# irmen/synthesizer

Measured on AMD Instinct MI355X. Metric: Msamples/sec mixed to stereo bus, 1024-voice additive @48kHz, higher is better.
Workload: dtype f64

## Files before the change

### synthesizer_amd/csrc/common.hpp

```cpp
#pragma once
#include <hip/hip_runtime.h>
#include <stdint.h>
#include <stddef.h>
#include <mutex>
#include <string>
#include "../../include/synthhip.h"

struct sh_buf {
    void*  ptr;
    size_t bytes;
    bool   owner;
    size_t cap = 0;
};

namespace sh {

struct PendingCombine {
    const void* parts = nullptr;
    uint32_t groups = 0, nframes = 0;
    void*    o32 = nullptr;
    void*    o64 = nullptr;
    void*    o16 = nullptr;
    double   scale = 0.0;
    const void* gen_valid = nullptr;
};

struct State {
    bool        initialized = false;
    int         device = -1;
    hipStream_t stream = nullptr;
    hipStream_t comm_stream = nullptr;
    hipEvent_t  ev_start = nullptr, ev_stop = nullptr;
    void*       scratch = nullptr;
    size_t      scratch_bytes = 0;
    int         last_mixdown_fused = 0;
    int         quantise_round = 0;
    int*        flag = nullptr;
    int*        flag_host = nullptr;
    void*       trig = nullptr;
    int         pending_total = 0;
    int         open_runs = 0;
    hipStream_t stream2 = nullptr;
    hipEvent_t  ev_join = nullptr;
    hipEvent_t  ev_aux = nullptr;
    hipEvent_t  ev_prep = nullptr;
    hipEvent_t  ev_sync = nullptr;
    bool        aux_busy = false;
};

State& state();

struct Knobs {
    bool no_speculation = false;
    bool no_overlap = false;
    bool no_split = false;
    bool no_seg = false;
    bool no_tiles = false;
    int  self = 0;
    bool no_ladder = false;
    bool no_period = false;
    int  period_chunks = 0;
    int  rt_cus = 0;
    int  seq_align = 0;
    bool no_small_pipeline = false;
    int  variant = 0;
    int  groups = 0;
    int  pool_fill = -1;
};
const Knobs& knobs();
void load_knobs();

struct Counters {
    uint64_t device_allocs = 0;
    uint64_t device_frees = 0;
    uint64_t stream_syncs = 0;
    uint64_t pool_hits = 0;
    uint64_t segmented_launches = 0, tiled_launches = 0, tiled_predicted = 0;
};
Counters& counters();
std::recursive_mutex& api_mutex();
#define SH_API_LOCK() std::lock_guard<std::recursive_mutex> sh_api_lock__(sh::api_mutex())
int  set_error(int code, const char* fmt, ...);
int  hip_error(hipError_t e, const char* what);
int  ensure_scratch(size_t bytes);
int  pool_alloc(size_t bytes, void** ptr, size_t* cap);
void pool_free(void* ptr, size_t cap);
void pool_trim();
struct Pooled {
    void*  ptr = nullptr;
    size_t cap = 0;
};
int  join_streams();
int  grow_pooled(Pooled& p, size_t bytes);
void release_pooled(Pooled& p);
int  flush_pending();
void free_render_buffers();
bool fold_owed_into(const void* p, size_t bytes);
inline bool has_pending() { return state().pending_total != 0 || state().aux_busy || state().open_runs != 0; }
int  bus_finalize_on(hipStream_t st, const double* in, size_t nvalues, float* out);

int bind_thread_to_device();
#define SH_REQUIRE_INIT_KEEP_PENDING()                                                 \
    SH_API_LOCK();                                                                     \
    do {                                                                               \
        if (!sh::state().initialized)                                                  \
            return sh::set_error(SH_ERR_NOTINIT, "sh_init() has not been called");     \
        { int rc_bind__ = sh::bind_thread_to_device(); if (rc_bind__) return rc_bind__; } \
    } while (0)

#define SH_REQUIRE_INIT()                                                              \
    SH_API_LOCK();                                                                     \
// ... 55 lines not shown
```

### synthesizer_amd/csrc/devmath.hpp

```cpp
#pragma once
#include <stdint.h>
#include <math.h>

#if defined(__HIPCC__)
#define SH_HD __host__ __device__ __forceinline__
#else
#define SH_HD static inline
#endif

namespace shm {

constexpr double PI_1 = 0x1.921fb54442d18p+1;
constexpr double PI_2 = 0x1.1a62633145c07p-53;
constexpr double PI_3 = -0x1.f1976b7ed8fbcp-109;
constexpr double INV_PI = 0.3183098861837907;
constexpr double PIO2_1 = 0x1.921fb54442d18p+0;
constexpr double PIO2_2 = 0x1.1a62633145c07p-54;
constexpr double PIO2_3 = -0x1.f1976b7ed8fbcp-110;
constexpr double TWO_OVER_PI = 0.6366197723675814;

SH_HD double flip_sign(double x, int odd) {
    union { double d; uint64_t u; } v;
    v.d = x;
    v.u ^= ((uint64_t)(odd & 1)) << 63;
// ... 56 lines not shown
    double fn = rint(t * TWO_OVER_PI);
    double r = fma(-fn, PIO2_1, t);
    r = fma(-fn, PIO2_2, r);
    r = fma(-fn, PIO2_3, r);
    int q = (int)fn;
    double z = r * r;
    double ps = -7.647163731819816e-13;
    ps = fma(ps, z, 1.6059043836821613e-10);
    ps = fma(ps, z, -2.505210838544172e-08);
    ps = fma(ps, z, 2.7557319223985893e-06);
    ps = fma(ps, z, -0.0001984126984126984);
    ps = fma(ps, z, 0.008333333333333333);
    ps = fma(ps, z, -0.16666666666666666);
    double sr = fma(r * z, ps, r);
    double pc = 4.779477332387385e-14;
    pc = fma(pc, z, -1.1470745597729725e-11);
    pc = fma(pc, z, 2.08767569878681e-09);
    pc = fma(pc, z, -2.755731922398589e-07);
    pc = fma(pc, z, 2.48015873015873e-05);
    pc = fma(pc, z, -0.001388888888888889);
    pc = fma(pc, z, 0.041666666666666664);
    pc = fma(pc, z, -0.5);
    double cr = fma(z, pc, 1.0);
    double s0 = (q & 1) ? cr : sr;
    double c0 = (q & 1) ? sr : cr;
    s = flip_sign(s0, (q >> 1) & 1);
    c = flip_sign(c0, ((q + 1) >> 1) & 1);
}

constexpr int    TRIG_N = 512;
constexpr double TRIG_STEP_1 = PI_1 / 256.0;
constexpr double TRIG_STEP_2 = PI_2 / 256.0;
constexpr double TRIG_STEP_3 = PI_3 / 256.0;
constexpr double TRIG_INV_STEP = 81.48733086305042;

struct sc_pair { double s, c; };

template <typename TablePtr>
SH_HD void sincos_tab(double t, TablePtr tab, double& s, double& c) {
    union { double d; uint64_t u; } m;
    m.d = fma(t, TRIG_INV_STEP, 6755399441055744.0);
    const double fk = m.d - 6755399441055744.0;
    double r = fma(-fk, TRIG_STEP_1, t);
    r = fma(-fk, TRIG_STEP_2, r);
    const uint32_t k = (uint32_t)m.u & (uint32_t)(TRIG_N - 1);
    const double S = tab[k].s, C = tab[k].c;
    const double z = r * r;
    const double sr = fma(r * z, fma(z, 0.008333333333333333, -0.16666666666666666), r);
    const double cr = fma(z, fma(z, 0.041666666666666664, -0.5), 1.0);
    s = fma(S, cr, C * sr);
    c = fma(C, cr, -(S * sr));
}

template <int N, typename TablePtr>
SH_HD void sincos_tab_n(const double (&t)[N], TablePtr tab, double (&s)[N], double (&c)[N]) {
    double r[N], S[N], C[N];
    for (int j = 0; j < N; ++j) {
        union { double d; uint64_t u; } m;
        m.d = fma(t[j], TRIG_INV_STEP, 6755399441055744.0);
        const double fk = m.d - 6755399441055744.0;
        const uint32_t k = (uint32_t)m.u & (uint32_t)(TRIG_N - 1);
        S[j] = tab[k].s;
        C[j] = tab[k].c;
        r[j] = fma(-fk, TRIG_STEP_2, fma(-fk, TRIG_STEP_1, t[j]));
    }
    double z[N], sr[N], cr[N];
    for (int j = 0; j < N; ++j) z[j] = r[j] * r[j];
    for (int j = 0; j < N; ++j) sr[j] = fma(z[j], 0.008333333333333333, -0.16666666666666666);
    for (int j = 0; j < N; ++j) cr[j] = fma(z[j], 0.041666666666666664, -0.5);
    for (int j = 0; j < N; ++j) sr[j] = fma(r[j] * z[j], sr[j], r[j]);
    for (int j = 0; j < N; ++j) cr[j] = fma(z[j], cr[j], 1.0);
    for (int j = 0; j < N; ++j) s[j] = fma(S[j], cr[j], C[j] * sr[j]);
    for (int j = 0; j < N; ++j) c[j] = fma(C[j], cr[j], -(S[j] * sr[j]));
}


SH_HD double saw_value(double t, double amp2, double bias) {
    double fl = floor(0.5 + t);
    return bias + amp2 * (t - fl);
}

SH_HD double square_value(double t, double amp, double bias) {
    double tr = trunc(t * 2.0);
    double h = tr * 0.5;
    bool odd = (h != rint(h)) && (fabs(tr) < 9007199254740992.0);
    return (odd ? -amp : amp) + bias;
}

SH_HD double pulse_value(double t, double pw, double amp, double bias) {
    double m = t - trunc(t);
    if (m < 0.0) m = m + 1.0;
    return ((m < pw) ? amp : -amp) + bias;
}

SH_HD double triangle_value(double t, double amp4, double bias) {
    double u = t + 0.75;
    double m = u - trunc(u);
    if (m < 0.0) m = m + 1.0;
    return amp4 * (fabs(m - 0.5) - 0.25) + bias;
}

}
```

### synthesizer_amd/csrc/osc_device.hpp

```cpp
#pragma once
#include "common.hpp"
#include "devmath.hpp"
#include "renderplan.hpp"
#include <type_traits>

namespace shosc {


constexpr uint32_t TILE_MAX_PIECES = 3;
struct alignas(64) TileRec {
    double t0, dt;
    double rc, rs;
    double ea0, ea1, eb0, eb1;
    double GL, GR;
    double tb[2], db[2];
    uint16_t split[2];
    uint16_t npieces;
    uint16_t corner;
    double pad_;
};
constexpr uint32_t TILE_WALK_PIECES = 16;
static_assert(sizeof(TileRec) == TILE_REC_BYTES && sizeof(TileRec) == 128 && offsetof(TileRec, GL) == 64 && offsetof(TileRec, tb) == 80 && offsetof(TileRec, split) == 112, "TileRec layout");
__device__ __forceinline__ double readlane_f64(double v, uint32_t src) {
    union { double d; int u[2]; } a, b;
// ... 988 lines not shown
                    if (SLOPED) {
                        const double ij = dl + (double)(f * 64);
                        accl[f] = fma(fma(ij, gls, gl), x, accl[f]);
                        accr[f] = fma(fma(ij, grs, gr), x, accr[f]);
                    } else {
                        accl[f] = fma(gl, x, accl[f]);
                        accr[f] = fma(gr, x, accr[f]);
                    }
                }
            }
        }
        return;
    }
#pragma unroll
    for (int h = 0; h < FPL; h += 2) {
        const bool two = h + 1 < FPL;
        double p0 = fma(poly[0], c0, poly[1]), p1 = fma(poly[0], c1, poly[1]);
#pragma unroll
        for (int u = 2; u < 16; ++u) {
            p0 = fma(p0, c0, poly[u]);
            if (two) p1 = fma(p1, c1, poly[u]);
        }
        const double x0 = p0 * s0;
        if (SLOPED) {
            const double i0 = dl + (double)(h * 64);
            accl[h] = fma(fma(i0, gls, gl), x0, accl[h]);
            accr[h] = fma(fma(i0, grs, gr), x0, accr[h]);
        } else {
            accl[h] = fma(gl, x0, accl[h]);
            accr[h] = fma(gr, x0, accr[h]);
        }
        if (two) {
            const double x1 = p1 * s1;
            if (SLOPED) {
                const double i1 = dl + (double)((h + 1) * 64);
                accl[h + 1 < FPL ? h + 1 : h] = fma(fma(i1, gls, gl), x1, accl[h + 1 < FPL ? h + 1 : h]);
                accr[h + 1 < FPL ? h + 1 : h] = fma(fma(i1, grs, gr), x1, accr[h + 1 < FPL ? h + 1 : h]);
            } else {
                accl[h + 1 < FPL ? h + 1 : h] = fma(gl, x1, accl[h + 1 < FPL ? h + 1 : h]);
                accr[h + 1 < FPL ? h + 1 : h] = fma(gr, x1, accr[h + 1 < FPL ? h + 1 : h]);
            }
        }
        if (h + 2 < FPL) {
            if (straddle) {
                shm::sincos_tab(theta(h + 2), trig, s0, c0);
                if (h + 3 < FPL) shm::sincos_tab(theta(h + 3), trig, s1, c1);
            } else {
                const double s2 = fma(k2, s1, -s0), c2 = fma(k2, c1, -c0);
                const double s3 = fma(k2, s2, -s1), c3 = fma(k2, c2, -c1);
                s0 = s2; c0 = c2; s1 = s3; c1 = c3;
            }
        }
    }
}

constexpr int TILE_WIN = 6;
template <typename V>
__device__ __forceinline__ V win_pick(const V (&a)[TILE_WIN], uint32_t r, V beyond) {
    V x = beyond;
#pragma unroll
    for (int k = 0; k < TILE_WIN; ++k) x = r == (uint32_t)k ? a[k] : x;
    return x;
}
__device__ __forceinline__ void prepare_tiles_wave(const BankPtrs& B, const TileSet& T, uint32_t nvoices, uint64_t start, uint32_t nframes,
                                                   uint32_t ntiles, uint32_t c, uint32_t run, const LaunchSet* recs = nullptr) {
    const uint32_t lane = threadIdx.x & 63, vi = c * 64 + lane;
    const size_t slots = (size_t)T.rec_chunks * 64;
    const uint32_t t_begin = run * TILES_PER_WAVE;
    if (t_begin >= ntiles) return;
    uint32_t t_end = t_begin + TILES_PER_WAVE;
    if (t_end > ntiles) t_end = ntiles;
    const bool valid = vi < nvoices;
    const uint64_t launch_end = start + (uint64_t)nframes;
    {
        const uint64_t span_lo = as_const(B.chunk_span)[2 * c], span_hi = as_const(B.chunk_span)[2 * c + 1];
        if (launch_end <= span_lo || start >= span_hi) {
            if (lane == 0)
                for (uint32_t t = t_begin; t < t_end; ++t) {
                    const size_t at = ((size_t)t * T.groups + c % T.groups) * T.mask_k + c / T.groups;
                    T.lean[at] = 0;
                    T.gen[at] = 0;
                }
            return;
        }
    }
    const sh_voice& v = B.voices[valid ? vi : 0];
    const int32_t v_kind = v.kind, v_dense = v.harm_dense, v_fm = v.fm_mode, v_flip = v.flip;
    const double v_bias = v.bias, amp = v.amplitude;
    const uint32_t off_c = v.seg_offset, cnt_c = v.seg_count, off_t = v.time_seg_offset, cnt_t = v.time_seg_count;
    const uint64_t onset = v.start_frame;
    const uint64_t e_na = v.env.n_attack_end, e_nd = v.env.n_decay_end, e_ns = v.env.n_sustain_end, e_nr = v.env.n_release_end;
    const double e_as = v.env.attack_slope, e_ds = v.env.decay_slope, e_sl = v.env.sustain_level, e_rs = v.env.release_slope;
    const int32_t e_on = v.env.enabled, e_tail = v.env.has_tail;
    const double bgl = (double)v.gain_l, bgr = (double)v.gain_r;
    const uint32_t hint = B.hint[valid ? vi : 0];
    asm volatile("" :: "v"(v_kind), "v"(v_dense), "v"(v_fm), "v"(v_flip), "v"(v_bias), "v"(amp), "v"(off_c), "v"(cnt_c), "v"(off_t), "v"(cnt_t),
                 "v"(onset), "v"(e_na), "v"(e_nd), "v"(e_ns), "v"(e_nr), "v"(e_as), "v"(e_ds), "v"(e_sl), "v"(e_rs), "v"(e_on), "v"(e_tail),
                 "v"(bgl), "v"(bgr), "v"(hint));
    const bool v_wave = v_kind == SH_SAWTOOTH || v_kind == SH_SQUARE || v_kind == SH_TRIANGLE || v_kind == SH_PULSE;
    const bool v_fm_sine = v_kind == SH_SINE && v_fm == SH_FM_SINE;
    const bool lean_capable = valid && v_bias == 0.0 && !v_flip &&
                              (v_fm_sine || (v_fm == SH_FM_NONE && ((v_kind == SH_HARMONICS && v_dense == 2) || v_kind == SH_SINE || v_wave)));
    const uint32_t rec_kind = v_fm_sine ? LEAN_FM : v_kind == SH_SAWTOOTH ? LEAN_SAW : v_kind == SH_SQUARE ? LEAN_SQUARE : v_kind == SH_TRIANGLE ? LEAN_TRIANGLE : v_kind == SH_PULSE ? LEAN_PULSE : LEAN_HARM;
    const bool fm = v_fm != SH_FM_NONE;
    const uint32_t off = fm ? off_t : off_c;
    const uint32_t cnt = fm ? cnt_t : cnt_c;
// ... 206 lines not shown
```

### synthesizer_amd/csrc/osc_render.hip

```cpp
#include "osc_host.hpp"
#include "osc_render_kernels.hpp"
#include "renderplan.hpp"
#include <stdlib.h>


namespace {

struct WriteRec { const char* lo; const char* hi; const sh_bank* owner; uint8_t streams; };
std::vector<WriteRec>& bank_writes() {
    static std::vector<WriteRec> v;
    return v;
}
bool overlaps_writes(const sh_bank* b, bool own, uint8_t streams, const void* p, size_t bytes) {
    if (!p) return false;
    const char* lo = (const char*)p;
    for (const WriteRec& r : bank_writes())
        if ((r.owner == b) == own && (!own || (r.streams & streams)) && lo < r.hi && r.lo < lo + bytes) return true;
    return false;
}
void note_write(const sh_bank* b, const void* p, size_t bytes, uint8_t stream_bit) {
    if (!p) return;
    const char* lo = (const char*)p;
    for (WriteRec& r : bank_writes())
        if (r.owner == b && r.lo == lo) { if (lo + bytes > r.hi) r.hi = lo + bytes; r.streams |= stream_bit; return; }
// ... 55 lines not shown
            const PendingCombine& pc = b->pending[k];
            const struct { const void* q; size_t n; } outs[3] = {{pc.o32, (size_t)pc.nframes * 8}, {pc.o64, (size_t)pc.nframes * 16}, {pc.o16, (size_t)pc.nframes * 4}};
            for (const auto& o : outs)
                if (o.q && lo < (const char*)o.q + o.n && (const char*)o.q < lo + bytes) return true;
        }
    return false;
}

int join_streams() {
    State& S = state();
    int rc = join_aux();
    if (rc) return rc;
    SH_HIP(hipEventRecord(S.ev_sync, S.stream));
    SH_HIP(hipStreamWaitEvent(S.stream2, S.ev_sync, 0));
    return SH_OK;
}

void free_render_buffers() {
    for (sh_bank* b : live_banks()) {
        for (int k = 0; k < 4; ++k) release_pooled(b->parts[k]);
        for (int k = 0; k < 2; ++k) {
            release_pooled(b->seg_block[k]);
            release_pooled(b->seg_scratch[k]);
            b->seg_cap[k] = 0;
        }
        release_pooled(b->gen_block);
        b->gen_segs = 0;
        for (int k = 0; k < sh_bank::NTILESETS; ++k) {
            release_pooled(b->tile_block[k]);
            b->tile_carved[k] = 0;
            b->tile_spec[k].valid = false;
        }
    }
}
}

struct RenderLaunch {
    sh_bank* b;
    hipStream_t st;
    shr::Call call;
    const shr::Shape& S;
    uint64_t next_start;
    uint32_t prep_wgs;
    bool use_aux;
    bool records_deferred;
    bool self_prepare;
    bool alone;
    LaunchSet cur, next;
    BusOut out;
    double2* parts;
    FoldIn fold;
    uint32_t* gen_valid;
    LaunchArgs args(const BankPtrs& P, const LaunchSet& set) const {
        return LaunchArgs{P, trig_table(), b->nvoices, S.vpg, set, call.start, call.nframes, self_prepare ? 1u : 0u, alone ? 1u : 0u};
    }
    NextArgs next_args(const LaunchSet& nx, uint32_t wgs) const { return NextArgs{nx, next_start, wgs}; }
};
static dim3 dim(shr::Grid g) { return dim3(g.x, g.y); }

static int launch_tiled(const RenderLaunch& L) {
    sh_bank* b = L.b;
    hipStream_t st = L.st;
    const shr::Shape& S = L.S;
    const shr::TiledGrids G = shr::tiled_grids(*b, S, L.call, L.next.launch != nullptr);
    int rc = SH_OK;
    const int ks = (int)(b->tile_count % sh_bank::NTILESETS);
    TileSet& T = b->tile_set[ks];
    sh_bank::TileSpec& sp = b->tile_spec[ks];
    BankPtrs P = ptrs(b);
    sh::counters().tiled_launches += 1;
    const bool predicted = shr::holds(sp, L.call, S.groups);
    if (predicted) sh::counters().tiled_predicted += 1;
    if (!predicted) {
        rc = grow_tile_set(b->tile_block[ks], T, b->tile_carved[ks], G.ntiles, b->nvoices, S.groups, (G.k1 - G.k0) * S.groups, st);
        if (rc) return rc;
        T.k0 = G.k0; T.k1 = G.k1;
        P.tiles = T;
        const LaunchSet own = launch_set(b, b->cur);
        rc = launch_prepare_tiles(st, P, T, b->nvoices, L.call.start, L.call.nframes, L.records_deferred ? &own : nullptr);
        if (rc) return rc;
    } else if (L.records_deferred) {
        rc = prepare_chunks_now(b, L.call.start, L.call.nframes, st);
        if (rc) return rc;
    }
    sp.valid = false;
    if (L.next.launch) {
        const int k2 = (int)((b->tile_count + 2) % sh_bank::NTILESETS);
        TileSet& T2 = b->tile_set[k2];
        rc = grow_tile_set(b->tile_block[k2], T2, b->tile_carved[k2], G.ntiles, b->nvoices, S.groups, (G.nk1 - G.nk0) * S.groups, st);
        if (rc) return rc;
        T2.k0 = G.nk0; T2.k1 = G.nk1;
        P.next_tiles = T2;
        P.next_ntiles = G.ntiles;
        P.next_tile_wgs = G.next_tile_wgs;
        b->tile_spec[k2] = sh_bank::TileSpec{true, L.next_start, L.call.nframes, S.groups};
    }
    P.tiles = T;
    const LaunchArgs A = L.args(P, L.cur);
    LaunchSet nx = L.next;
    if (!G.next_in_kernel) nx.launch = nullptr;
    const NextArgs N = L.next_args(nx, G.behind);
    if (G.merged) {
        if (b->tile_waveforms) hipLaunchKernelGGL((k_render_tiles<4, 8, 3, true, true>), dim(G.tiles), dim3(256), 0, st, A, N, L.fold, L.parts, L.gen_valid);
        else hipLaunchKernelGGL((k_render_tiles<4, 8, 3, false, true>), dim(G.tiles), dim3(256), 0, st, A, N, L.fold, L.parts, L.gen_valid);
    } else {
        if (b->tile_waveforms) hipLaunchKernelGGL((k_render_tiles<4, 8, 3, true, false>), dim(G.tiles), dim3(256), 0, st, A, N, L.fold, L.parts, L.gen_valid);
        else hipLaunchKernelGGL((k_render_tiles<4, 8, 4, false, false>), dim(G.tiles), dim3(256), 0, st, A, N, L.fold, L.parts, L.gen_valid);
// ... 305 lines not shown
```

### synthesizer_amd/csrc/osc_render_kernels.hpp

```cpp
#pragma once
#include "osc_device.hpp"
#include <type_traits>

namespace shosc {
struct BusOut {
    float2*   bus32;
    double2*  bus64;
    uint32_t* pcm16;
    double    pcm_scale;
};
struct FoldIn {
    const double2*  parts;
    const uint32_t* gen_valid;
    BusOut          out;
    uint32_t*       self;
};
struct LaunchArgs {
    BankPtrs              B;
    const shm::sc_pair*   trig_g;
    uint32_t              nvoices, voices_per_group;
    LaunchSet             cur;
    uint64_t              start;
    uint32_t              nframes;
    uint32_t              self_prepare;
    uint32_t              alone;
};
struct NextArgs {
    LaunchSet next;
    uint64_t  next_start;
    uint32_t  prep_wgs;
};
int launch_render_lean(int var, int kinds, bool seg, dim3 grid, hipStream_t st, const LaunchArgs& A, const NextArgs& N, const FoldIn& F, double2* parts);
int launch_render_combined(int var, int mode, dim3 grid, hipStream_t st, const LaunchArgs& A, const NextArgs& N, const FoldIn& F, double2* parts, const BusOut& out);
}

namespace {


#ifdef SH_DIAG
constexpr uint32_t DIAG_WAVES = 4096, DIAG_SLOTS = 10;
__device__ uint64_t g_diag[4 * DIAG_WAVES * DIAG_SLOTS];
__device__ __forceinline__ void diag_stamp(uint64_t start_, uint32_t nframes_, uint32_t slot) {
    const uint32_t w = (blockIdx.y * gridDim.x + blockIdx.x) * (blockDim.x >> 6) + (threadIdx.x >> 6);
    if ((threadIdx.x & 63) == 0 && w < DIAG_WAVES) {
        const uint32_t bank = (uint32_t)((double)start_ * __builtin_amdgcn_rcp((double)nframes_) + 0.5);
        uint64_t* d = g_diag + ((size_t)(bank & 3) * DIAG_WAVES + w) * DIAG_SLOTS;
        d[slot] = __builtin_amdgcn_s_memrealtime();
        if (slot == 0) {
            uint32_t hw, xcc;
            asm volatile("s_getreg_b32 %0, hwreg(HW_REG_HW_ID)" : "=s"(hw));
            asm volatile("s_getreg_b32 %0, hwreg(HW_REG_XCC_ID)" : "=s"(xcc));
            d[6] = (uint64_t)hw | ((uint64_t)xcc << 32);
            d[7] = __builtin_amdgcn_s_memtime();
            d[9] = ((uint64_t)gridDim.x << 32) | gridDim.y;
        }
        if (slot == 5) d[8] = __builtin_amdgcn_s_memtime();
    }
}
__device__ uint64_t g_diag2[64 * 8];
#define SH_STAMP(A_, slot) diag_stamp((A_).start, (A_).nframes, slot)
#else
#define SH_STAMP(A_, slot) ((void)0)
#endif

struct TileCtx {
    uint32_t lane, wave;
    uint32_t grp, ngroups;
    uint32_t tile_index, tile0, tile_last, nfr;
    uint32_t seg_off;
    uint64_t st0;
    uint32_t c0, c1;
    LaunchSet set;
    uint32_t alone;
};

template <int FPL>
__device__ __forceinline__ void tile_bounds(TileCtx& T) {
    T.tile0 = T.tile_index * (64 * FPL);
    T.tile_last = T.tile0 + 64 * FPL - 1;
    if (T.tile_last > T.nfr - 1) T.tile_last = T.nfr - 1;
}

__device__ __forceinline__ void group_chunks(TileCtx& T, const LaunchArgs& A) {
    T.c0 = (T.grp * A.voices_per_group) / 64;
    T.c1 = ((T.grp + 1) * A.voices_per_group + 63) / 64;
    const uint32_t nchunks = (A.nvoices + 63) / 64;
    if (T.c1 > nchunks) T.c1 = nchunks;
}

template <int FPL>
__device__ __forceinline__ TileCtx plain_tile(const LaunchArgs& A, uint32_t bx, uint32_t grp, uint32_t ngroups) {
    TileCtx T;
    T.lane = threadIdx.x & 63;
    T.wave = __builtin_amdgcn_readfirstlane(threadIdx.x >> 6);
    T.grp = grp;
    T.ngroups = ngroups;
    T.tile_index = bx;
    T.nfr = A.nframes;
    T.seg_off = 0;
    T.st0 = A.start;
    T.set = A.cur;
    T.alone = A.alone;
    tile_bounds<FPL>(T);
    group_chunks(T, A);
    return T;
}

template <int FPL>
__device__ __forceinline__ void enter_segment(TileCtx& T, const LaunchArgs& A) {
    uint32_t sidx = 0;
    for (;;) {
        const uint32_t n_s = A.B.seg_first[sidx + 1] - A.B.seg_first[sidx];
        const uint32_t tiles_s = (n_s + 64 * FPL - 1) / (64 * FPL);
        if (T.tile_index < tiles_s || sidx + 1 >= A.B.nseg) break;
        T.tile_index -= tiles_s;
        ++sidx;
    }
    T.seg_off = A.B.seg_first[sidx];
    T.nfr = A.B.seg_first[sidx + 1] - T.seg_off;
    T.st0 = A.start + T.seg_off;
    T.set = segment_set(A.cur, sidx, A.nvoices);
    tile_bounds<FPL>(T);
}

template <int FPL>
__device__ __forceinline__ void build_frames(const TileCtx& T, uint32_t lane_, uint32_t (&i)[FPL], double (&di)[FPL]) {
#pragma unroll
    for (int j = 0; j < FPL; ++j) {
        const uint32_t raw = T.tile0 + j * 64 + lane_;
        i[j] = raw < T.nfr ? raw : T.nfr - 1;
        di[j] = (double)i[j];
    }
}

__device__ __forceinline__ void load_trig(shm::sc_pair* trig, const shm::sc_pair* __restrict__ trig_g, uint32_t nthreads) {
    for (uint32_t k = threadIdx.x; k < shm::TRIG_N; k += nthreads) trig[k] = trig_g[k];
    __syncthreads();
}

__device__ __forceinline__ uint32_t groups_of_grid(uint32_t prep_wgs) {
    return gridDim.y - (prep_wgs ? (prep_wgs + gridDim.x - 1) / gridDim.x : 0u);
}
__device__ __forceinline__ bool prep_rows_lists(const LaunchArgs& A, const NextArgs& N, uint32_t ngroups) {
    if (!N.prep_wgs || blockIdx.y < ngroups) return false;
    const uint32_t unit = (blockIdx.y - ngroups) * gridDim.x + blockIdx.x;
    if (N.next.launch && unit < N.prep_wgs && threadIdx.x < 64) {
        __builtin_amdgcn_s_setprio(3);
        if (unit < (A.nvoices + 63) / 64) prepare_chunk(A.B, N.next, unit, A.nvoices, N.next_start, A.nframes);
    }
    return true;
}
template <bool MERGED>
__device__ __forceinline__ int prep_rows_tiles(const LaunchArgs& A, const NextArgs& N, uint32_t ngroups, uint32_t& gen_unit) {
    if (!N.prep_wgs || blockIdx.y < ngroups) return 0;
    const uint32_t unit = (blockIdx.y - ngroups) * gridDim.x + blockIdx.x;
// ... 231 lines not shown
        r[j] = fma(-fk, shm::TRIG_STEP_2, fma(-fk, shm::TRIG_STEP_1, t[j]));
    }
    double z[N], sr[N], cr[N];
#pragma unroll
    for (int j = 0; j < N; ++j) z[j] = r[j] * r[j];
#pragma unroll
    for (int j = 0; j < N; ++j) sr[j] = fma(z[j], s5, -0.16666666666666666);
#pragma unroll
    for (int j = 0; j < N; ++j) cr[j] = fma(z[j], 0.041666666666666664, -0.5);
#pragma unroll
    for (int j = 0; j < N; ++j) sr[j] = fma(r[j] * z[j], sr[j], r[j]);
#pragma unroll
    for (int j = 0; j < N; ++j) cr[j] = fma(z[j], cr[j], 1.0);
#pragma unroll
    for (int j = 0; j < N; ++j) s[j] = fma(S[j], cr[j], C[j] * sr[j]);
}

#ifndef SH_FM_Q
#define SH_FM_Q 2
#endif
template <int FPL, bool BIASED, bool LINEAR, int QMAX = SH_FM_Q, typename TimeFn>
__device__ __forceinline__ void lean_fm_frames(const double (&poly)[16], double lfo_a_rel, double startd, double lfo_d, double lfo_K, double lfo_C0,
                                               double lrc, double lrs, double di0, TimeFn time,
                                               double t_first, double t_step, TrigTab trig, double (&out)[FPL]) {
    const double frequency = poly[0], f_inc = poly[2], lfo_bias = poly[7];
    double magic = 6755399441055744.0, s5 = 0.008333333333333333, phase0 = poly[1];
    asm volatile("" : "+v"(magic), "+v"(s5), "+v"(phase0));
    double ls0, lc0;
    shm::sincos_tab(fma(di0, lfo_d, lfo_a_rel), trig, ls0, lc0);
    double lc1 = fma(lc0, lrc, -(ls0 * lrs));
    const double lk2 = lrc + lrc;
    double tj = t_first;
    constexpr int Q = FPL < QMAX ? FPL : QMAX;
#pragma unroll
    for (int h = 0; h < FPL; h += Q) {
        double th[Q], sn[Q];
#pragma unroll
        for (int jj = 0; jj < Q; ++jj) {
            const int j = h + jj;
            const double Ln = BIASED ? fma(lfo_K, lfo_C0 - lc0, lfo_bias * (startd + (di0 + (double)(j * 64)))) : lfo_K * (lfo_C0 - lc0);
            const double tt = LINEAR ? tj : time(j);
            th[jj] = frequency * tt + fma(f_inc, Ln, phase0);
            if (LINEAR) tj = tj + t_step;
            const double lc2 = fma(lk2, lc1, -lc0);
            lc0 = lc1;
            lc1 = lc2;
        }
        sin_tab_n<Q>(th, trig, magic, s5, sn);
#pragma unroll
        for (int jj = 0; jj < Q; ++jj) out[h + jj] = sn[jj];
    }
}

template <int WAVES, int FPL, int KINDS, bool SEG>
__device__ __forceinline__ void lean_lists(const TileCtx& T, uint32_t& first, TrigTab trig, double (&accl)[FPL], double (&accr)[FPL]) {
    const uint32_t lane = T.lane, tile0 = T.tile0, tile_last = T.tile_last;
    for (uint32_t c = T.c0; c < T.c1; ++c) {
        const uint32_t nfast = as_const(T.set.counts)[4 * c];
        auto entry = [&](auto cls_, const FastRec SH_CONST_AS* q, uint32_t p) __attribute__((always_inline)) {
            constexpr int CLS = decltype(cls_)::value;
            (void)p;
#ifdef SH_DIAG2
            const bool d2on = blockIdx.x == 1 && blockIdx.y == 1 && T.wave == 0 && c == T.c0 + 1;
            uint64_t d2t[5] = {0, 0, 0, 0, 0};
            if (d2on) d2t[0] = __builtin_amdgcn_s_memtime();
#endif
            const double gl = q->gain_l, gr = q->gain_r;
            const uint32_t remain = q->remain, kind = q->kind;
            const uint32_t lsplit = CLS == LEAN_K_FM ? q->pad1 : 0xFFFFFFFFu;
            const double ta = q->t_base, da = q->dt, rca = q->rot_c, rsa = q->rot_s;
            double poly[16];
#pragma unroll
            for (int u = 0; u < 16; ++u) poly[u] = q->poly[u];
            if constexpr (CLS == LEAN_K_FM) asm volatile("" :: "s"(lsplit));
            asm volatile("" :: "s"(gl), "s"(gr), "s"(remain), "s"(kind), "s"(ta), "s"(da), "s"(rca), "s"(rsa),
                         "s"(poly[0]), "s"(poly[1]), "s"(poly[2]), "s"(poly[3]), "s"(poly[4]), "s"(poly[5]),
                         "s"(poly[6]), "s"(poly[7]), "s"(poly[8]), "s"(poly[9]), "s"(poly[10]), "s"(poly[11]), "s"(poly[12]),
                         "s"(poly[13]), "s"(poly[14]), "s"(poly[15]));
            const uint32_t i0 = tile0 + lane;
            const double di0 = (double)i0;
            double t_base = ta, dt = da, rc = rca, rs = rsa, off = 0.0, tb = ta, db = da, ob = 0.0;
            bool straddle = false;
            if constexpr (SEG) {
                const double tb2 = q->t0_b, db2 = q->dt_b, ob2 = q->off_b, rcb = q->rot_c_b, rsb = q->rot_s_b;
                asm volatile("" :: "s"(tb2), "s"(db2), "s"(ob2), "s"(rcb), "s"(rsb));
                if (remain != 0xFFFFFFFFu && tile_last >= remain) {
                    tb = tb2; db = db2; ob = ob2;
                    straddle = tile0 < remain;
                    if (!straddle) { t_base = tb; dt = db; rc = rcb; rs = rsb; off = ob; }
                }
            } else
            if (remain != 0xFFFFFFFFu && tile_last >= remain) {
                tb = q->t0_b; db = q->dt_b; ob = q->off_b;
                const double rcb = q->rot_c_b, rsb = q->rot_s_b;
                straddle = tile0 < remain;
                if (!straddle) { t_base = tb; dt = db; rc = rcb; rs = rsb; off = ob; }
            }
            const LaneTheta theta{di0, t_base, dt, off, ta, da, tb, db, ob, i0, remain, straddle};
            if constexpr (CLS == LEAN_K_FM) {
                double sn[FPL];
                double l_a = poly[3], l_d = poly[4], l_K = poly[5], l_C = poly[6], l_rc = poly[8], l_rs = poly[9];
                if (tile0 >= lsplit) { l_a = poly[11]; l_d = poly[12]; l_K = poly[13]; l_C = poly[14]; l_rc = poly[15]; l_rs = q->pad2; }
                if (straddle) {
                    lean_fm_frames<FPL, false, false>(poly, l_a, poly[10], l_d, l_K, l_C, l_rc, l_rs, di0, theta, 0.0, 0.0, trig, sn);
                } else {
                    const double t_first = fma(di0 - off, dt, t_base), t_step = 64.0 * dt;
                    lean_fm_frames<FPL, false, true>(poly, l_a, poly[10], l_d, l_K, l_C, l_rc, l_rs, di0, theta, t_first, t_step, trig, sn);
                }
#pragma unroll
                for (int j = 0; j < FPL; ++j) {
                    accl[j] = fma(gl, sn[j], accl[j]);
// ... 24 lines not shown
                    lean_harm_frames<FPL, true>(s0, c0, s1, c1, rc + rc, straddle, theta, trig, poly, gl, gr, accl, accr, gls, grs, di0);
                } else {
                    lean_harm_frames<FPL>(s0, c0, s1, c1, rc + rc, straddle, theta, trig, poly, gl, gr, accl, accr);
                }
#ifdef SH_DIAG2
                asm volatile("" : "+v"(accl[FPL - 1]), "+v"(accr[FPL - 1]), "+v"(accl[0]));
                if (d2on) {
                    d2t[4] = __builtin_amdgcn_s_memtime();
                    const uint32_t it = (p - first) / WAVES;
                    if (lane == 0 && it < 12) {
#pragma unroll
                        for (int k_ = 0; k_ < 5; ++k_) g_diag2[it * 8 + k_] = d2t[k_];
                    }
                }
#endif
                return;
            }
            if constexpr (CLS == LEAN_K_REST) {
            if (kind == LEAN_SINE) {
                double s0, c0, s1, c1;
                shm::sincos_tab(theta(0), trig, s0, c0);
                if (straddle) {
                    if (FPL > 1) shm::sincos_tab(theta(1), trig, s1, c1); else { s1 = s0; c1 = c0; }
                } else {
                    s1 = fma(s0, rc, c0 * rs);
                }
                const double k2 = rc + rc;
#pragma unroll
                for (int j = 0; j < FPL; ++j) {
                    accl[j] = fma(gl, s0, accl[j]);
                    accr[j] = fma(gr, s0, accr[j]);
                    if (j + 1 < FPL) {
                        double s2;
                        if (straddle) { if (j + 2 < FPL) shm::sincos_tab(theta(j + 2), trig, s2, c1); else s2 = 0.0; }
                        else s2 = fma(k2, s1, -s0);
                        s0 = s1;
                        s1 = s2;
                    }
                }
                return;
            }
#pragma unroll
            for (int j = 0; j < FPL; ++j) {
                const double th = theta(j);
                const double x = kind == LEAN_SAW ? shm::saw_value(th, 2.0, 0.0)
                               : kind == LEAN_SQUARE ? shm::square_value(th, 1.0, 0.0)
                               : kind == LEAN_TRIANGLE ? shm::triangle_value(th, 4.0, 0.0)
                               : shm::pulse_value(th, poly[0], 1.0, 0.0);
                accl[j] = fma(gl, x, accl[j]);
                accr[j] = fma(gr, x, accr[j]);
            }
            }
        };
        const FastRec SH_CONST_AS* q = as_const(T.set.fast) + c * 64 + first;
        uint32_t p = first;
        if constexpr (KINDS == LEAN_K_ALL) {
            const uint32_t runs = as_const(T.set.counts)[4 * c + 3];
            const uint32_t end_harm = runs & 0xFFu, end_fm = end_harm + ((runs >> 8) & 0xFFu);
            for (; p < end_harm; p += WAVES, q += WAVES) entry(std::integral_constant<int, LEAN_K_HARM>{}, q, p);
            for (; p < end_fm; p += WAVES, q += WAVES) entry(std::integral_constant<int, LEAN_K_FM>{}, q, p);
            for (; p < nfast; p += WAVES, q += WAVES) entry(std::integral_constant<int, LEAN_K_REST>{}, q, p);
        } else {
            const uint32_t span = (T.c1 - T.c0) * 64u;
            for (; p < nfast; p += WAVES, q += WAVES) {
                if (T.alone) {
                    const uint32_t at8 = ((c - T.c0) * 64u + p) * 8u;
                    if (at8 < 4 * span) __builtin_amdgcn_s_setprio(3);
                    else if (at8 < 6 * span) __builtin_amdgcn_s_setprio(2);
                    else if (at8 < 7 * span) __builtin_amdgcn_s_setprio(1);
                    else __builtin_amdgcn_s_setprio(0);
                }
                entry(std::integral_constant<int, KINDS>{}, q, p);
            }
        }
        first = p - nfast;
    }
}

template <int WAVES, int FPL>
__device__ __forceinline__ void general_lists(const LaunchArgs& A, const TileCtx& T, uint32_t& first, uint32_t nsub, const uint32_t (&i)[FPL],
                                              const double (&di)[FPL], TrigTab trig, double (&accl)[FPL], double (&accr)[FPL]) {
    for (uint32_t c = T.c0; c < T.c1; ++c) {
        const uint32_t ngen = as_const(T.set.counts)[4 * c + 1];
        const uint32_t SH_CONST_AS* idx = as_const(T.set.gen_idx) + c * 64;
        const uint32_t step = WAVES * nsub;
        uint32_t p = first;
        uint32_t vi_next = p < ngen ? idx[p] : 0u;
        for (; p < ngen; p += step) {
            const uint32_t vi = vi_next;
            vi_next = p + step < ngen ? idx[p + step] : 0u;
            const VoiceRegs r = load_record(as_const(T.set.launch) + vi);
            general_voice<FPL>(r, T.set.fm + vi, A.B, A.B.voices + vi, T.st0, T.tile0, T.nfr, i, di, trig, accl, accr);
        }
        first = p - ngen;
    }
}

__device__ __forceinline__ uint32_t general_count(const uint32_t* counts, uint32_t c0, uint32_t c1) {
    uint32_t total = 0;
    for (uint32_t c = c0; c < c1; ++c) total += as_const(counts)[4 * c + 1];
    return total;
}

enum { TILE_RUN_HARM = 0, TILE_RUN_FM = 1, TILE_RUN_REST = 2 };
template <int WAVES, int FPL, bool WAVEFORMS>
__device__ __forceinline__ void tiles_lean(const BankPtrs& B, const TileCtx& T, TrigTab trig, double (&accl)[FPL], double (&accr)[FPL]) {
    static_assert(64 * FPL == TILE_FRAMES, "the lean kernel's tile is the tile of the classification");
    const uint32_t lane = T.lane, ngroups = T.ngroups, tile_index = T.tile_index;
    const size_t slots = (size_t)B.tiles.rec_chunks * 64;
    const TileRec SH_CONST_AS* trow = as_const(B.tiles.recs) + (size_t)tile_index * slots;
    const uint32_t kw = B.tiles.k1 - B.tiles.k0, nmask = ngroups * kw, stride = ngroups * WAVES;
    const uint64_t* __restrict__ lrow = B.tiles.lean + (size_t)tile_index * (ngroups * B.tiles.mask_k);
    uint32_t firstp = __builtin_amdgcn_readfirstlane(T.grp * WAVES + T.wave);
    for (uint32_t base = 0; base < nmask; base += 64) {
        const uint32_t mi = base + lane;
        const uint64_t mymask = mi < nmask ? lrow[(mi / kw) * B.tiles.mask_k + B.tiles.k0 + mi % kw] : 0ull;
        const uint64_t have0 = __ballot(mymask != 0ull);
        uint64_t have = ((uint64_t)(uint32_t)__builtin_amdgcn_readfirstlane((int)(uint32_t)(have0 >> 32)) << 32) |
                        (uint64_t)(uint32_t)__builtin_amdgcn_readfirstlane((int)(uint32_t)have0);
        while (have) {
            const uint32_t src = (uint32_t)__builtin_ctzll(have);
            have &= have - 1;
            const uint64_t cmask = ((uint64_t)(uint32_t)__builtin_amdgcn_readlane((int)(uint32_t)(mymask >> 32), (int)src) << 32) |
                                   (uint64_t)(uint32_t)__builtin_amdgcn_readlane((int)(uint32_t)mymask, (int)src);
            const uint32_t npairs = (uint32_t)cmask;
            const uint32_t idx = base + src;
            const uint32_t c = idx / kw + (B.tiles.k0 + idx % kw) * ngroups;
            auto pair = [&](auto cls_, const TileRec SH_CONST_AS* q) __attribute__((always_inline)) {
// ... 210 lines not shown
    for (uint32_t base = 0; base < nmask; base += 64) {
        const uint32_t mi = base + (threadIdx.x & 63);
        const uint64_t mine = mi < nmask ? grow[(mi / kw) * B.tiles.mask_k + B.tiles.k0 + mi % kw] : 0ull;
        any = any || __ballot(mine != 0ull) != 0ull;
    }
    return any;
}
template <int WAVES, int FPL>
__device__ __forceinline__ void tiles_general(const LaunchArgs& A, const TileCtx& T, uint32_t gen_part, const uint32_t (&i)[FPL], const double (&di)[FPL],
                                              TrigTab trig, double (&accl)[FPL], double (&accr)[FPL]) {
    const BankPtrs& B = A.B;
    const uint32_t kw = B.tiles.k1 - B.tiles.k0, nmask = B.tiles.groups * kw;
    const uint64_t* __restrict__ grow = B.tiles.gen + (size_t)(T.tile0 / TILE_FRAMES) * (B.tiles.groups * B.tiles.mask_k);
    uint32_t ord = 0;
    for (uint32_t base = 0; base < nmask; base += 64) {
        const uint32_t mi = base + T.lane;
        const uint64_t mine = mi < nmask ? grow[(mi / kw) * B.tiles.mask_k + B.tiles.k0 + mi % kw] : 0ull;
        uint64_t have = __ballot(mine != 0ull);
        while (have) {
            const uint32_t src = (uint32_t)__builtin_ctzll(have);
            have &= have - 1;
            uint64_t m = ((uint64_t)(uint32_t)__builtin_amdgcn_readlane((int)(uint32_t)(mine >> 32), (int)src) << 32) |
                         (uint64_t)(uint32_t)__builtin_amdgcn_readlane((int)(uint32_t)mine, (int)src);
            const uint32_t idx = base + src;
            const uint32_t c = idx / kw + (B.tiles.k0 + idx % kw) * B.tiles.groups;
            while (m) {
                const uint32_t bit = (uint32_t)__builtin_ctzll(m);
                m &= m - 1;
                if ((ord++ % (uint32_t)(WAVES * GEN_SPLIT)) != T.wave * GEN_SPLIT + gen_part) continue;
                const uint32_t vi = c * 64 + bit;
                const VoiceRegs r = load_record(as_const(T.set.launch) + vi);
                general_voice<FPL>(r, T.set.fm + vi, B, B.voices + vi, T.st0, T.tile0, T.nfr, i, di, trig, accl, accr);
            }
        }
    }
}
template <int WAVES, int FPL>
__device__ __forceinline__ void zero_tile(double2* __restrict__ plane, uint32_t tile_first, uint32_t nfr) {
    for (uint32_t f = threadIdx.x; f < 64 * FPL; f += WAVES * 64) {
        const uint32_t raw = tile_first + f;
        if (raw < nfr) plane[raw] = make_double2(0.0, 0.0);
    }
}

template <int FPL>
__device__ __forceinline__ void clear_acc(double (&accl)[FPL], double (&accr)[FPL]) {
#pragma unroll
    for (int j = 0; j < FPL; ++j) {
        accl[j] = 0.0;
        accr[j] = 0.0;
    }
}

template <int WAVES, int FPL, int MINW, int KINDS, bool SEG>
__global__ __launch_bounds__(WAVES * 64, MINW) void k_render_lean(LaunchArgs A, NextArgs N, FoldIn F, double2* __restrict__ parts) {
    SH_STAMP(A, 0);
    const uint32_t ngroups = groups_of_grid(N.prep_wgs);
    if (prep_rows_lists(A, N, ngroups)) return;
    fold_previous<WAVES, FPL>(F, ngroups, A.nframes, blockIdx.x);
    if constexpr (!SEG) {
        if (A.self_prepare) prepare_own_group<WAVES>(A, blockIdx.y);
    }
    SH_STAMP(A, 1);
    __shared__ double red[WAVES][2][64 * red_rows(FPL)];
    __shared__ shm::sc_pair trig[shm::TRIG_N];
    load_trig(trig, A.trig_g, WAVES * 64);
    SH_STAMP(A, 2);
    TileCtx T = plain_tile<FPL>(A, blockIdx.x, blockIdx.y, ngroups);
    if constexpr (SEG) enter_segment<FPL>(T, A);
    double accl[FPL], accr[FPL];
    clear_acc(accl, accr);
    uint32_t first = T.wave;
    lean_lists<WAVES, FPL, KINDS, SEG>(T, first, trig, accl, accr);
    SH_STAMP(A, 3);
    SH_STAMP(A, 4);
    reduce_store<WAVES, FPL>(red, T, accl, accr, parts + (size_t)T.grp * A.nframes, T.seg_off, BusOut{}, !SEG && F.self != nullptr);
    SH_STAMP(A, 5);
    if constexpr (!SEG) {
        if (F.self) fold_own_tile<WAVES, FPL>(F, ngroups, A.nframes, blockIdx.x, reinterpret_cast<uint32_t*>(&red[0][0][0]));
    }
}

enum { GEN_LISTS = 0, GEN_SEG = 1, GEN_TILES = 2 };
template <int WAVES, int FPL, int MINW, int KIND>
__global__ __launch_bounds__(WAVES * 64, MINW) void k_render_general(LaunchArgs A, double2* __restrict__ parts, uint32_t* __restrict__ gen_valid) {
    const BankPtrs& B = A.B;
    uint32_t gen_part = 0, sub = 0, nsub = 1;
    bool to_scratch = false;
    TileCtx T;
    if constexpr (KIND == GEN_TILES) {
        __builtin_amdgcn_s_setprio(3);
        gen_part = blockIdx.x % GEN_SPLIT;
        const uint32_t bx = blockIdx.x / GEN_SPLIT;
        if (bx * (64 * FPL) >= A.nframes) return;
        if (bx == 0 && gen_part == 0 && threadIdx.x < B.tiles.groups) gen_valid[threadIdx.x] = threadIdx.x < GEN_SPLIT ? 1u : 0u;
        double2* plane = parts + (size_t)(B.tiles.groups + gen_part) * A.nframes;
        if (!tile_has_general<WAVES>(B, (bx * (64 * FPL)) / TILE_FRAMES)) {
            zero_tile<WAVES, FPL>(plane, bx * (64 * FPL), A.nframes);
            return;
        }
        T = plain_tile<FPL>(A, bx, 0, B.tiles.groups);
    } else if constexpr (KIND == GEN_LISTS) {
        T = plain_tile<FPL>(A, blockIdx.x, blockIdx.y, gridDim.y);
        const uint32_t total = general_count(A.cur.counts, T.c0, T.c1);
        if (blockIdx.x == 0 && threadIdx.x == 0) gen_valid[blockIdx.y] = total ? 1u : 0u;
        if (total == 0) return;
    } else {
        T = plain_tile<FPL>(A, blockIdx.x, blockIdx.y, gridDim.y);
        const uint32_t tiles_0 = (B.seg_first[1] - B.seg_first[0] + 64 * FPL - 1) / (64 * FPL);
        if (T.tile_index < tiles_0 * B.gen_sub) {
            sub = T.tile_index % B.gen_sub;
            T.tile_index /= B.gen_sub;
            nsub = B.gen_sub;
            to_scratch = true;
        } else {
            T.tile_index -= tiles_0 * (B.gen_sub - 1);
        }
        enter_segment<FPL>(T, A);
        if (!to_scratch && general_count(T.set.counts, T.c0, T.c1) == 0) {
            zero_tile<WAVES, FPL>(parts + (size_t)(T.ngroups + T.grp) * A.nframes + T.seg_off, T.tile0, T.nfr);
            return;
        }
    }
    __shared__ double red[WAVES][2][64 * red_rows(FPL)];
    __shared__ shm::sc_pair trig[shm::TRIG_N];
    load_trig(trig, A.trig_g, WAVES * 64);
// ... 135 lines not shown
```

### synthesizer_amd/csrc/runtime.hip

```cpp
#include "common.hpp"
#include <stdarg.h>
#include <stdio.h>
#include <string.h>
#include <math.h>
#include <stdlib.h>
#include <vector>
#include <unordered_map>

namespace sh {

static thread_local char g_err[512] = "";

State& state() {
    static State s;
    return s;
}

static Knobs g_knobs;
const Knobs& knobs() { return g_knobs; }
Counters& counters() {
    static Counters c;
    return c;
}

void load_knobs() {
    auto flag = [](const char* name) { const char* e = getenv(name); return e && e[0] == '1'; };
    auto num = [](const char* name, long dflt) { const char* e = getenv(name); return e ? atol(e) : dflt; };
    Knobs k;
    k.no_speculation = flag("SYNTHHIP_NO_SPECULATION");
    k.no_overlap = flag("SYNTHHIP_NO_OVERLAP");
    k.no_split = flag("SYNTHHIP_NO_SPLIT");
    k.no_seg = flag("SYNTHHIP_NO_SEG");
    k.no_tiles = flag("SYNTHHIP_NO_TILES");
    k.no_small_pipeline = flag("SYNTHHIP_NO_SMALL_PIPELINE");
    k.self = (int)num("SYNTHHIP_SELF", 0);
    k.rt_cus = (int)num("SYNTHHIP_RT_CUS", 0);
    k.no_ladder = flag("SYNTHHIP_NO_LADDER");
    k.no_period = flag("SYNTHHIP_NO_PERIOD");
    k.period_chunks = (int)num("SYNTHHIP_PERIOD_CHUNKS", 0);
    k.seq_align = (int)num("SYNTHHIP_SEQ_ALIGN", 0);
    k.variant = (int)num("SYNTHHIP_VARIANT", 0);
    k.groups = (int)num("SYNTHHIP_GROUPS", 0);
    k.pool_fill = (int)num("SYNTHHIP_POOL_FILL", -1);
    g_knobs = k;
}

int bind_thread_to_device() {
    const int want = state().device;
    int cur = -1;
    if (hipGetDevice(&cur) != hipSuccess || cur != want) SH_HIP(hipSetDevice(want));
    return SH_OK;
}

std::recursive_mutex& api_mutex() {
    static std::recursive_mutex m;
    return m;
}

int set_error(int code, const char* fmt, ...) {
    va_list ap;
    va_start(ap, fmt);
    vsnprintf(g_err, sizeof(g_err), fmt, ap);
    va_end(ap);
    return code;
}

int hip_error(hipError_t e, const char* what) {
    int code = (e == hipErrorOutOfMemory) ? SH_ERR_NOMEM : SH_ERR_HIP;
    return set_error(code, "%s: %s", what, hipGetErrorString(e));
}

namespace {
struct Pool {
    std::unordered_map<size_t, std::vector<void*>> free_;
    size_t cached = 0;
    static constexpr size_t LIMIT = size_t(16) << 30;
};
Pool g_pool;

size_t size_class(size_t bytes) {
    if (bytes <= 256) return 256;
    size_t p = 256;
    while (p < bytes) p <<= 1;
    const size_t step = p >> 4;
    return (bytes + step - 1) / step * step;
}
}

int pool_alloc(size_t bytes, void** ptr, size_t* cap) {
    const size_t c = size_class(bytes);
// ... 359 lines not shown
```

Measured before the change: 1.386 million.

## Software-pipeline voice loop in lean harmonic kernel to overlap next-voice seeding

Adds a pipelined voice loop for the lean polynomial-harmonics render kernel (FPL=16, MINW=3, no segments). While the current voice's frames are synthesized, it prefetches the next voice records and computes the next voice's sine/cosine seed, split into a head and a table-lookup tail. Scheduling barriers and asm register pins interleave the seed latency with the recurrence and polynomial math. This targets the per-voice serialization of record loads and seeding, at the cost of higher register pressure and more complex control flow. It is on by default and can be turned off with an environment knob.

```diff
diff --git a/synthesizer_amd/csrc/common.hpp b/synthesizer_amd/csrc/common.hpp
--- a/synthesizer_amd/csrc/common.hpp
+++ b/synthesizer_amd/csrc/common.hpp
@@ -57,6 +57,7 @@
     bool no_seg = false;
     bool no_tiles = false;
     int  self = 0;
+    bool no_voice_pipeline = false;
     bool no_ladder = false;
     bool no_period = false;
     int  period_chunks = 0;
diff --git a/synthesizer_amd/csrc/devmath.hpp b/synthesizer_amd/csrc/devmath.hpp
--- a/synthesizer_amd/csrc/devmath.hpp
+++ b/synthesizer_amd/csrc/devmath.hpp
@@ -132,6 +132,27 @@
     c = fma(C, cr, -(S * sr));
 }
 
+struct sincos_head { uint32_t k; double sr, cr; };
+SH_HD sincos_head sincos_tab_head(double t) {
+    union { double d; uint64_t u; } m;
+    m.d = fma(t, TRIG_INV_STEP, 6755399441055744.0);
+    const double fk = m.d - 6755399441055744.0;
+    double r = fma(-fk, TRIG_STEP_1, t);
+    r = fma(-fk, TRIG_STEP_2, r);
+    sincos_head h;
+    h.k = (uint32_t)m.u & (uint32_t)(TRIG_N - 1);
+    const double z = r * r;
+    h.sr = fma(r * z, fma(z, 0.008333333333333333, -0.16666666666666666), r);
+    h.cr = fma(z, fma(z, 0.041666666666666664, -0.5), 1.0);
+    return h;
+}
+template <typename TablePtr>
+SH_HD void sincos_tab_tail(const sincos_head& h, TablePtr tab, double& s, double& c) {
+    const double S = tab[h.k].s, C = tab[h.k].c;
+    s = fma(S, h.cr, C * h.sr);
+    c = fma(C, h.cr, -(S * h.sr));
+}
+
 template <int N, typename TablePtr>
 SH_HD void sincos_tab_n(const double (&t)[N], TablePtr tab, double (&s)[N], double (&c)[N]) {
     double r[N], S[N], C[N];
diff --git a/synthesizer_amd/csrc/osc_device.hpp b/synthesizer_amd/csrc/osc_device.hpp
--- a/synthesizer_amd/csrc/osc_device.hpp
+++ b/synthesizer_amd/csrc/osc_device.hpp
@@ -1064,6 +1064,86 @@
             }
         }
     }
+}
+
+struct LeanSeed { double s0, c0, s1, c1, k2; };
+struct LeanSeedIn { double th0, rc, rs, k2; };
+template <typename Theta>
+__device__ __forceinline__ LeanSeed lean_seed(Theta theta, TrigTab trig, double rc, double rs) {
+    LeanSeed n;
+    shm::sincos_tab(theta(0), trig, n.s0, n.c0);
+    n.s1 = fma(n.s0, rc, n.c0 * rs);
+    n.c1 = fma(n.c0, rc, -(n.s0 * rs));
+    n.k2 = rc + rc;
+    return n;
+}
+template <int FPL, typename Arrived, typename Mid>
+__device__ __forceinline__ LeanSeed lean_harm_frames_piped(const LeanSeed& cur, const double (&poly)[16], const double& gl, const double& gr,
+                                                           double (&accl)[FPL], double (&accr)[FPL],
+                                                           const LeanSeedIn next, TrigTab trig, Arrived arrived, Mid mid) {
+    constexpr int CH = SH_LEAN_CH, HB = FPL > 8 ? CH : (FPL < 8 ? FPL : 8);
+    static_assert(CH > 2 && FPL % HB == 0 && HB % CH == 0 && HB >= 2, "frames per lane: a multiple of the chains, in halves of eight");
+    shm::sincos_head head = shm::sincos_tab_head(next.th0);
+    LeanSeed nx;
+    const double k2 = cur.k2;
+    double s[HB], c[HB], p1 = 0.0, tab_s = 0.0, tab_c = 0.0;
+#pragma unroll
+    for (int h0 = 0; h0 < FPL; h0 += HB) {
+        if (h0 == 0) {
+            s[0] = cur.s0; c[0] = cur.c0;
+            s[1] = cur.s1; c[1] = cur.c1;
+#pragma unroll
+            for (int j = 2; j < HB; ++j) {
+                s[j] = fma(k2, s[j - 1], -s[j - 2]);
+                c[j] = fma(k2, c[j - 1], -c[j - 2]);
+            }
+            asm volatile("" : "+v"(head.k), "+v"(head.sr), "+v"(head.cr), "+v"(s[HB - 2]), "+v"(c[HB - 2]), "+v"(s[HB - 1]), "+v"(c[HB - 1]));
+            arrived();
+            p1 = poly[1];
+            asm volatile("" : "+v"(p1));
+            tab_s = trig[head.k].s; tab_c = trig[head.k].c;
+        } else {
+            const double sa = s[HB - 2], sb = s[HB - 1], ca = c[HB - 2], cb = c[HB - 1];
+            s[0] = fma(k2, sb, -sa); c[0] = fma(k2, cb, -ca);
+            s[1] = fma(k2, s[0], -sb); c[1] = fma(k2, c[0], -cb);
+#pragma unroll
+            for (int j = 2; j < HB; ++j) {
+                s[j] = fma(k2, s[j - 1], -s[j - 2]);
+                c[j] = fma(k2, c[j - 1], -c[j - 2]);
+            }
+        }
+#pragma unroll
+        for (int h = 0; h < HB; h += CH) {
+            double p[CH];
+#pragma unroll
+            for (int jj = 0; jj < CH; ++jj) p[jj] = fma(poly[0], c[h + jj], p1);
+#pragma unroll
+            for (int u = 2; u < 16; ++u) {
+#pragma unroll
+                for (int jj = 0; jj < CH; ++jj) p[jj] = fma(p[jj], c[h + jj], poly[u]);
+            }
+#pragma unroll
+            for (int jj = 0; jj < CH; ++jj) {
+                const double x = p[jj] * s[h + jj];
+                const int f = h0 + h + jj;
+                accl[f] = fma(gl, x, accl[f]);
+                accr[f] = fma(gr, x, accr[f]);
+            }
+        }
+        if (h0 == 0) {
+            asm volatile("" : "+v"(accl[HB - 1]), "+v"(accr[HB - 1]));
+            __builtin_amdgcn_sched_barrier(0);
+            nx.s0 = fma(tab_s, head.cr, tab_c * head.sr);
+            nx.c0 = fma(tab_c, head.cr, -(tab_s * head.sr));
+            nx.s1 = fma(nx.s0, next.rc, nx.c0 * next.rs);
+            nx.c1 = fma(nx.c0, next.rc, -(nx.s0 * next.rs));
+            nx.k2 = next.k2;
+            asm volatile("" : "+v"(nx.s0), "+v"(nx.c0), "+v"(nx.s1), "+v"(nx.c1));
+            mid();
+            __builtin_amdgcn_sched_barrier(0);
+        }
+    }
+    return nx;
 }
 
 constexpr int TILE_WIN = 6;
diff --git a/synthesizer_amd/csrc/osc_render.hip b/synthesizer_amd/csrc/osc_render.hip
--- a/synthesizer_amd/csrc/osc_render.hip
+++ b/synthesizer_amd/csrc/osc_render.hip
@@ -131,7 +131,7 @@
     FoldIn fold;
     uint32_t* gen_valid;
     LaunchArgs args(const BankPtrs& P, const LaunchSet& set) const {
-        return LaunchArgs{P, trig_table(), b->nvoices, S.vpg, set, call.start, call.nframes, self_prepare ? 1u : 0u, alone ? 1u : 0u};
+        return LaunchArgs{P, trig_table(), b->nvoices, S.vpg, set, call.start, call.nframes, self_prepare ? 1u : 0u, alone ? 1u : 0u, sh::knobs().no_voice_pipeline ? 0u : 1u};
     }
     NextArgs next_args(const LaunchSet& nx, uint32_t wgs) const { return NextArgs{nx, next_start, wgs}; }
 };
diff --git a/synthesizer_amd/csrc/osc_render_kernels.hpp b/synthesizer_amd/csrc/osc_render_kernels.hpp
--- a/synthesizer_amd/csrc/osc_render_kernels.hpp
+++ b/synthesizer_amd/csrc/osc_render_kernels.hpp
@@ -24,6 +24,7 @@
     uint32_t              nframes;
     uint32_t              self_prepare;
     uint32_t              alone;
+    uint32_t              piped;
 };
 struct NextArgs {
     LaunchSet next;
@@ -72,6 +73,7 @@
     uint32_t c0, c1;
     LaunchSet set;
     uint32_t alone;
+    uint32_t piped;
 };
 
 template <int FPL>
@@ -101,6 +103,7 @@
     T.st0 = A.start;
     T.set = A.cur;
     T.alone = A.alone;
+    T.piped = A.piped;
     tile_bounds<FPL>(T);
     group_chunks(T, A);
     return T;
@@ -438,11 +441,102 @@
     }
 }
 
-template <int WAVES, int FPL, int KINDS, bool SEG>
+template <int WAVES, int FPL, typename Entry>
+__device__ __forceinline__ void lean_lists_piped(const TileCtx& T, uint32_t& first, TrigTab trig, double (&accl)[FPL], double (&accr)[FPL],
+                                                 uint32_t& c, uint32_t& lane_of_entry, Entry entry) {
+    if (T.c0 >= T.c1) return;
+    const uint32_t tile0 = T.tile0, tile_last = T.tile_last, c1 = T.c1;
+    uint64_t counts_u = (uint64_t)T.set.counts, fast_u = (uint64_t)T.set.fast;
+    asm volatile("" : "+s"(counts_u), "+s"(fast_u));
+    const uint32_t SH_CONST_AS* counts = as_const((const uint32_t*)counts_u);
+    const FastRec SH_CONST_AS* fast = as_const((const FastRec*)fast_u);
+    struct Walk { uint32_t c, p, nfast, nfast_nx; };
+    auto count_of = [&](uint32_t ch) { return counts[4 * (ch < c1 ? ch : c1 - 1)]; };
+    auto settle = [&](Walk& w) {
+        while (w.c < c1 && w.p >= w.nfast) { w.p -= w.nfast; ++w.c; w.nfast = w.nfast_nx; w.nfast_nx = count_of(w.c + 1); }
+    };
+    auto step = [&](Walk w) { w.p += WAVES; settle(w); return w; };
+    const uint32_t span = (c1 - T.c0) * 64u;
+    const double di0 = (double)(tile0 + T.lane);
+    struct Fields { double ta, da, rc, rs; uint32_t remain; };
+    auto fields = [&](const FastRec SH_CONST_AS* q) { return Fields{q->t_base, q->dt, q->rot_c, q->rot_s, q->remain}; };
+    auto one_piece = [&](uint32_t remain) { return remain == 0xFFFFFFFFu || tile_last < remain; };
+    auto theta_of = [&](const Fields& f) { return LaneTheta{di0, f.ta, f.da, 0.0, f.ta, f.da, f.ta, f.da, 0.0, tile0 + T.lane, f.remain, false}; };
+
+    struct Place { uint32_t c, p; };
+    Walk look{T.c0, first, count_of(T.c0), count_of(T.c0 + 1)};
+    settle(look);
+    Place w{look.c, look.p};
+    auto seed_in = [&](const Fields& f) {
+        LeanSeedIn in{theta_of(f)(0), f.rc, f.rs, f.rc + f.rc};
+        asm volatile("" : "+v"(in.th0), "+v"(in.rc), "+v"(in.rs), "+v"(in.k2));
+        return in;
+    };
+    LeanSeed sd{};
+    LeanSeedIn in1{};
+    bool warm = false, warm1 = false;
+    while (w.c < c1) {
+        const FastRec SH_CONST_AS* q = fast + w.c * 64 + w.p;
+        if (T.alone) {
+            const uint32_t at8 = ((w.c - T.c0) * 64u + w.p) * 8u;
+            if (at8 < 4 * span) __builtin_amdgcn_s_setprio(3);
+            else if (at8 < 6 * span) __builtin_amdgcn_s_setprio(2);
+            else if (at8 < 7 * span) __builtin_amdgcn_s_setprio(1);
+            else __builtin_amdgcn_s_setprio(0);
+        }
+        if (!warm) {
+            look = step(Walk{w.c, w.p, count_of(w.c), count_of(w.c + 1)});
+            const Fields f0 = fields(q);
+            const Fields f1 = fields(look.c < c1 ? fast + look.c * 64 + look.p : q);
+            if (!one_piece(f0.remain)) {
+                c = w.c;
+                asm volatile("" : "+v"(lane_of_entry));
+                entry(std::integral_constant<int, LEAN_K_HARM>{}, q, w.p);
+                w = Place{look.c, look.p};
+                continue;
+            }
+            sd = lean_seed(theta_of(f0), trig, f0.rc, f0.rs);
+            in1 = seed_in(f1);
+            warm1 = look.c < c1 && one_piece(f1.remain);
+        }
+        const Place n1{look.c, look.p};
+        look = step(look);
+        const bool more2 = look.c < c1;
+        const FastRec SH_CONST_AS* q2 = more2 ? fast + look.c * 64 + look.p : q;
+        const double gl = q->gain_l, gr = q->gain_r;
+        double poly[16];
+#pragma unroll
+        for (int u = 0; u < 16; ++u) poly[u] = q->poly[u];
+        const Fields f2 = fields(q2);
+        const uint32_t touch = reinterpret_cast<const uint32_t SH_CONST_AS*>(&q2->poly[2])[0];
+        bool warm2 = false;
+        auto arrived = [&]() __attribute__((always_inline)) {
+            __builtin_amdgcn_sched_barrier(0);
+            asm volatile("" :: "s"(gl), "s"(gr), "s"(f2.ta), "s"(f2.da), "s"(f2.rc), "s"(f2.rs), "s"(f2.remain), "s"(touch),
+                         "s"(poly[0]), "s"(poly[1]), "s"(poly[2]), "s"(poly[3]), "s"(poly[4]), "s"(poly[5]),
+                         "s"(poly[6]), "s"(poly[7]), "s"(poly[8]), "s"(poly[9]), "s"(poly[10]), "s"(poly[11]), "s"(poly[12]),
+                         "s"(poly[13]), "s"(poly[14]), "s"(poly[15]));
+            __builtin_amdgcn_sched_barrier(0);
+        };
+        auto mid = [&]() __attribute__((always_inline)) {
+            in1 = seed_in(f2);
+            warm2 = more2 && one_piece(f2.remain);
+        };
+        sd = lean_harm_frames_piped<FPL>(sd, poly, gl, gr, accl, accr, in1, trig, arrived, mid);
+        warm = warm1;
+        warm1 = warm2;
+        w = n1;
+    }
+    first = w.p;
+}
+
+template <int WAVES, int FPL, int KINDS, bool SEG, bool PIPED = false>
 __device__ __forceinline__ void lean_lists(const TileCtx& T, uint32_t& first, TrigTab trig, double (&accl)[FPL], double (&accr)[FPL]) {
-    const uint32_t lane = T.lane, tile0 = T.tile0, tile_last = T.tile_last;
-    for (uint32_t c = T.c0; c < T.c1; ++c) {
-        const uint32_t nfast = as_const(T.set.counts)[4 * c];
+    static_assert(!PIPED || (KINDS == LEAN_K_HARM && !SEG), "the pipelined voice loop: steady polynomial-Harmonics blocks");
+    const uint32_t tile0 = T.tile0, tile_last = T.tile_last;
+    uint32_t lane = T.lane;
+    uint32_t c = T.c0;
+    {
         auto entry = [&](auto cls_, const FastRec SH_CONST_AS* q, uint32_t p) __attribute__((always_inline)) {
             constexpr int CLS = decltype(cls_)::value;
             (void)p;
@@ -573,6 +667,11 @@
             }
             }
         };
+        if constexpr (PIPED) {
+            if (T.piped) { lean_lists_piped<WAVES, FPL>(T, first, trig, accl, accr, c, lane, entry); return; }
+        }
+        for (; c < T.c1; ++c) {
+        const uint32_t nfast = as_const(T.set.counts)[4 * c];
         const FastRec SH_CONST_AS* q = as_const(T.set.fast) + c * 64 + first;
         uint32_t p = first;
         if constexpr (KINDS == LEAN_K_ALL) {
@@ -595,6 +694,7 @@
             }
         }
         first = p - nfast;
+        }
     }
 }
 
@@ -911,6 +1011,7 @@
     }
 }
 
+constexpr bool lean_piped(int fpl, int minw, int kinds, bool seg) { return fpl == 16 && minw == 3 && kinds == LEAN_K_HARM && !seg; }
 template <int WAVES, int FPL, int MINW, int KINDS, bool SEG>
 __global__ __launch_bounds__(WAVES * 64, MINW) void k_render_lean(LaunchArgs A, NextArgs N, FoldIn F, double2* __restrict__ parts) {
     SH_STAMP(A, 0);
@@ -930,7 +1031,7 @@
     double accl[FPL], accr[FPL];
     clear_acc(accl, accr);
     uint32_t first = T.wave;
-    lean_lists<WAVES, FPL, KINDS, SEG>(T, first, trig, accl, accr);
+    lean_lists<WAVES, FPL, KINDS, SEG, lean_piped(FPL, MINW, KINDS, SEG)>(T, first, trig, accl, accr);
     SH_STAMP(A, 3);
     SH_STAMP(A, 4);
     reduce_store<WAVES, FPL>(red, T, accl, accr, parts + (size_t)T.grp * A.nframes, T.seg_off, BusOut{}, !SEG && F.self != nullptr);
diff --git a/synthesizer_amd/csrc/runtime.hip b/synthesizer_amd/csrc/runtime.hip
--- a/synthesizer_amd/csrc/runtime.hip
+++ b/synthesizer_amd/csrc/runtime.hip
@@ -36,6 +36,7 @@
     k.self = (int)num("SYNTHHIP_SELF", 0);
     k.rt_cus = (int)num("SYNTHHIP_RT_CUS", 0);
     k.no_ladder = flag("SYNTHHIP_NO_LADDER");
+    k.no_voice_pipeline = flag("SYNTHHIP_NO_VOICE_PIPELINE");
     k.no_period = flag("SYNTHHIP_NO_PERIOD");
     k.period_chunks = (int)num("SYNTHHIP_PERIOD_CHUNKS", 0);
     k.seq_align = (int)num("SYNTHHIP_SEQ_ALIGN", 0);
```

After: 1.343 million. -3.1%, worse.
